# czbiohub-sf/yogo

Hardware: AMD Instinct MI355X
Metric: training images/sec (772x1032 gray) (higher is better)
Workload: dtype bf16; 1 GPU; BASELINE configs[2]: full train step (fwd+loss+bwd+clamp+AdamW), base_model, 772x1032x1 uint8, 7 classes; per_gpu_batch=128, global_batch=128, parallelism=dp1

## Files before the change

include/yogo_hip.h:

```cpp
#ifndef YOGO_HIP_H
#define YOGO_HIP_H

#include <stddef.h>

#ifdef __cplusplus
extern "C" {
#endif

typedef void* yogo_stream_t;

const char* yogo_hip_last_error(void);
int yogo_hip_abi_version(void);
int yogo_hip_launch_log(int enable);
int yogo_hip_launch_log_read(char* buf, size_t cap, size_t* needed);


int yogo_conv_packed_bytes(int Cin, int Cout, int ksize, int stride, int mode, size_t* bytes);
int yogo_conv_pack_f32(const float* w_oihw, float* packed, int Cin, int Cout, int ksize, int stride, int mode,
                       yogo_stream_t stream);
int yogo_conv2d_fwd_stats_shape(int B, int Cin, int Cout, int IH, int IW, int ksize, int stride, int* rows, int* mpad);
int yogo_conv2d_fwd_f32(const float* in, const float* packed, const float* bias, float* out, float* out_pre,
                        const float* chan_scale, float* stats_part, int B, int Cin, int Cout, int IH, int IW, int ksize,
                        int stride, int act, yogo_stream_t stream);
int yogo_conv2d_dgrad_f32(const float* dy, const float* packed_dgrad, float* dx, const float* act_ref, int ref_act,
// ... 22 lines not shown
                const float* beta, int act, float* dgamma, float* dbeta, float* part, float* sums, int B, int C, int HW,
                int training, float clip, yogo_stream_t stream);
int yogo_partials_reduce(float* part, int rows, int N, float clip, float* out, yogo_stream_t stream);
int yogo_channel_sum(const float* g, int B, int C, int HW, float clip, float* out, yogo_stream_t stream);

int yogo_decode_fwd(const float* raw, float* out, const float* cxs, const float* cys, int B, int P, int Sy, int Sx,
                    float anchor_w, float anchor_h, float width_multiplier, float height_multiplier, int inference,
                    yogo_stream_t stream);
int yogo_decode_bwd(const float* raw, const float* out, const float* gout, float* graw, int B, int P, int Sy, int Sx,
                    int inference, yogo_stream_t stream);

int yogo_decode_bwd_bf16(const float* raw, const float* out, const float* gout, void* graw8c, int B, int P, int Sy, int Sx,
                         int inference, yogo_stream_t stream);

int yogo_loss_workspace_bytes(int B, int Sy, int Sx, size_t* bytes);
int yogo_loss_fwd_bwd(const float* pred, const float* label, float* grad, float* loss_out, void* workspace, int B, int P,
                      int Sy, int Sx, float no_obj_weight, float iou_weight, float classify_weight, float label_smoothing,
                      yogo_stream_t stream);

int yogo_decode_loss_bwd_bf16(const float* raw, const float* label, const float* cxs, const float* cys, void* graw8c, float* loss_out,
                              void* workspace, int B, int P, int Sy, int Sx, float anchor_w, float anchor_h, float width_multiplier,
                              float height_multiplier, float no_obj_weight, float iou_weight, float classify_weight,
                              float label_smoothing, yogo_stream_t stream);

int yogo_format_preds_workspace_bytes(int B, int Sy, int Sx, size_t* bytes);
int yogo_format_preds_batched(const float* pred, float* out_rows, long long* out_cells, int* out_count, void* workspace,
                              int B, int P, int Sy, int Sx, int cap, double obj_thresh, double iou_thresh, int box_format,
                              double min_class_confidence_threshold, yogo_stream_t stream);
int yogo_decode_format_preds_batched(const float* raw, const float* cxs, const float* cys, float* out_rows, long long* out_cells,
                                     int* out_count, void* workspace, int B, int P, int Sy, int Sx, int cap, float anchor_w,
                                     float anchor_h, float width_multiplier, float height_multiplier, int inference,
                                     double obj_thresh, double iou_thresh, int box_format, double min_class_confidence_threshold,
                                     yogo_stream_t stream);
int yogo_head1x1_decode_fwd_bf16(const void* x, const void* packed, const float* bias, float* out, const float* cxs, const float* cys,
                                 int B, int Cin, int P, int Sy, int Sx, float anchor_w, float anchor_h, float width_multiplier,
                                 float height_multiplier, int inference, yogo_stream_t stream);

int yogo_match_workspace_bytes(int B, int Sy, int Sx, int cap, size_t* bytes);
int yogo_match_preds_labels_batched(const float* rows, const int* counts, const float* labels, int* meta, int* pair_label,
                                    int* pair_pred, int* un_label, int* un_pred, float* lab_out, void* workspace, int B, int P, int Sy,
                                    int Sx, int cap, yogo_stream_t stream);
int yogo_match_gather(const float* rows, const float* lab_out, const int* meta, const int* pair_label, const int* pair_pred,
                      const int* un_label, const int* un_pred, float* preds, float* labels, float* missed, float* extra, int B, int P,
                      int cap, long long K, long long Km, long long Ke, yogo_stream_t stream);
int yogo_metrics_state_layout(int C, int T, int nbins, long long* offsets);
int yogo_metrics_accumulate(const float* rows, const float* lab_out, const int* meta, const int* pair_label, const int* pair_pred,
// ... 182 lines not shown
```

yogo_amd/csrc/decode_loss.hip:

```cpp
#include "head_math.h"

#define MAX_CLASSES 64

__global__ __launch_bounds__(256) void decode_fwd_kernel(const float* __restrict__ raw, float* __restrict__ out,
                                                         const float* __restrict__ cxs, const float* __restrict__ cys,
                                                         float inv_sx, float inv_sy, float anchor_w, float anchor_h,
                                                         float wmul, float hmul, int P, int cells, int inference) {
  const int b = blockIdx.y;
  const int cell = blockIdx.x * 256 + threadIdx.x;
  if (cell >= cells) return;
  const float* r = raw + (size_t)b * P * cells + cell;
  float* o = out + (size_t)b * P * cells + cell;
  const float t0 = r[0], t1 = r[(size_t)cells], t2 = r[(size_t)2 * cells], t3 = r[(size_t)3 * cells], t4 = r[(size_t)4 * cells];
  o[0] = hm_centre(inv_sx, t0, cxs[cell]);
  o[(size_t)cells] = hm_centre(inv_sy, t1, cys[cell]);
  o[(size_t)2 * cells] = hm_size(anchor_w, t2, wmul);
  o[(size_t)3 * cells] = hm_size(anchor_h, t3, hmul);
  o[(size_t)4 * cells] = hm_sigmoid(t4);
  const int C = P - 5;
  if (inference) {
    float mx, sum;
    hm_softmax_terms(r, cells, P, mx, sum);
    for (int c = 0; c < C; ++c) o[(size_t)(5 + c) * cells] = hm_softmax(r[(size_t)(5 + c) * cells], mx, sum);
  } else {
// ... 27 lines not shown
  }
}

__global__ __launch_bounds__(256) void decode_bwd_bf16_kernel(const float* __restrict__ raw, const float* __restrict__ out,
                                                              const float* __restrict__ gout, hm_u32x4* __restrict__ g8, float inv_sx,
                                                              float inv_sy, int P, int Pb, int cells, int inference) {
  const int b = blockIdx.y;
  const int cell = blockIdx.x * 256 + threadIdx.x;
  if (cell >= cells) return;
  const size_t base = (size_t)b * P * cells + cell;
  const float* r = raw + base;
  const float* o = out + base;
  const float* g = gout + base;
  const float dot = inference ? hm_softmax_bwd_dot(g, o, cells, P) : 0.f;
  const float s0 = hm_sigmoid(r[0]), s1 = hm_sigmoid(r[(size_t)cells]), s4 = o[(size_t)4 * cells];
  hm_store_bf16_8c(g8, b, cell, cells, P, Pb, [&](int ch) {
    const float gv = g[(size_t)ch * cells];
    if (ch == 0) return hm_centre_bwd(gv, inv_sx, s0);
    if (ch == 1) return hm_centre_bwd(gv, inv_sy, s1);
    if (ch == 2 || ch == 3) return hm_size_bwd(gv, r[(size_t)ch * cells], o[(size_t)ch * cells]);
    if (ch == 4) return hm_obj_bwd(gv, s4);
    return inference ? hm_softmax_bwd(gv, o[(size_t)ch * cells], dot) : gv;
  });
}

struct LossWeights {
  float no_obj_weight, iou_weight, classify_weight, label_smoothing, inv_batch;
};
static LossWeights loss_weights(float no_obj_weight, float iou_weight, float classify_weight, float label_smoothing, int B) {
  return {no_obj_weight, iou_weight, classify_weight, label_smoothing, 1.0f / (float)B};
}

struct LossParams {
  const float* pred;
  const float* label;
  float* grad;
  float* part;
  int B, P, cells;
  LossWeights w;
};

__global__ __launch_bounds__(256) void yogo_loss_kernel(const LossParams p) {
  const int b = blockIdx.y;
  const int cell = blockIdx.x * 256 + threadIdx.x;
  const int cells = p.cells;
  const int C = p.P - 5;
  float l_iou = 0.f, l_obj = 0.f, l_cls = 0.f;
  if (cell < cells) {
    const float* pr = p.pred + (size_t)b * p.P * cells + cell;
    const float* lb = p.label + (size_t)b * 6 * cells + cell;
    float* gr = p.grad + (size_t)b * p.P * cells + cell;
    const float m = lb[0];
    l_obj = hm_obj_term(pr[(size_t)4 * cells], m, p.w.no_obj_weight, p.w.inv_batch, gr[(size_t)4 * cells]);
// ... 3 lines not shown
                           p.w.iou_weight * p.w.inv_batch, g0, g1, g2, g3);
    gr[0] = g0;
    gr[(size_t)cells] = g1;
    gr[(size_t)2 * cells] = g2;
    gr[(size_t)3 * cells] = g3;
    if (m != 0.f) {
      HmCeTerms ce;
      l_cls = hm_ce_cell(pr, cells, lb[(size_t)5 * cells], p.P, m, p.w.label_smoothing, p.w.classify_weight, p.w.inv_batch, ce);
      for (int c = 0; c < C; ++c) gr[(size_t)(5 + c) * cells] = hm_ce_grad(pr[(size_t)(5 + c) * cells], c, C, p.w.label_smoothing, ce);
    } else {
      for (int c = 0; c < C; ++c) gr[(size_t)(5 + c) * cells] = 0.f;
    }
  }
  hm_block_sum3(l_iou, l_obj, l_cls, p.part, b);
}

struct FusedParams {
  const float* raw;
  const float* label;
  const float *cxs, *cys;
  hm_u32x4* g8;
  float* part;
  int B, P, Pb, cells;
  float inv_sx, inv_sy, anchor_w, anchor_h, wmul, hmul;
  LossWeights w;
};

__global__ __launch_bounds__(256) void decode_loss_bwd_bf16_kernel(const FusedParams p) {
  const int b = blockIdx.y;
  const int cell = blockIdx.x * 256 + threadIdx.x;
  const int cells = p.cells;
  const int C = p.P - 5;
  float l_iou = 0.f, l_obj = 0.f, l_cls = 0.f;
  if (cell < cells) {
    const float* r = p.raw + (size_t)b * p.P * cells + cell;
    const float* lb = p.label + (size_t)b * 6 * cells + cell;
    const float t0 = r[0], t1 = r[(size_t)cells], t2 = r[(size_t)2 * cells], t3 = r[(size_t)3 * cells], t4 = r[(size_t)4 * cells];
    const float s0 = hm_sigmoid(t0), s1 = hm_sigmoid(t1);
    const float pcx = hm_centre(p.inv_sx, t0, p.cxs[cell]);
    const float pcy = hm_centre(p.inv_sy, t1, p.cys[cell]);
    const float pw = hm_size(p.anchor_w, t2, p.wmul);
    const float ph = hm_size(p.anchor_h, t3, p.hmul);
    const float po = hm_sigmoid(t4);
    const float m = lb[0];
    float gobj, g0 = 0.f, g1 = 0.f, g2 = 0.f, g3 = 0.f;
    l_obj = hm_obj_term(po, m, p.w.no_obj_weight, p.w.inv_batch, gobj);
    HmCeTerms ce{};
    if (m != 0.f) {
      l_iou = hm_ciou_cell(pcx, pcy, pw, ph, lb, cells, p.w.iou_weight * p.w.inv_batch, g0, g1, g2, g3);
      l_cls = hm_ce_cell(r, cells, lb[(size_t)5 * cells], p.P, m, p.w.label_smoothing, p.w.classify_weight, p.w.inv_batch, ce);
    }
    hm_store_bf16_8c(p.g8, b, cell, cells, p.P, p.Pb, [&](int ch) {
      if (ch == 0) return hm_centre_bwd(g0, p.inv_sx, s0);
      if (ch == 1) return hm_centre_bwd(g1, p.inv_sy, s1);
      if (ch == 2) return hm_size_bwd(g2, t2, pw);
      if (ch == 3) return hm_size_bwd(g3, t3, ph);
      if (ch == 4) return hm_obj_bwd(gobj, po);
      return m != 0.f ? hm_ce_grad(r[(size_t)ch * cells], ch - 5, C, p.w.label_smoothing, ce) : 0.f;
    });
  }
  hm_block_sum3(l_iou, l_obj, l_cls, p.part, b);
}

__global__ __launch_bounds__(256) void yogo_loss_finalize_kernel(const float* __restrict__ part, int rows, float iou_weight,
                                                                 float classify_weight, float inv_batch,
                                                                 float* __restrict__ out) {
  __shared__ double sh[3][4];
  double s[3] = {0.0, 0.0, 0.0};
  for (int r = threadIdx.x; r < rows; r += 256)
    for (int k = 0; k < 3; ++k) s[k] += (double)part[(size_t)r * 3 + k];
  const int lane = threadIdx.x & 63, wave = threadIdx.x >> 6;
  for (int k = 0; k < 3; ++k) {
    s[k] = wave_sum_d(s[k]);
    if (lane == 0) sh[k][wave] = s[k];
  }
  __syncthreads();
  if (threadIdx.x == 0) {
    const float iou = (float)(iou_weight * (sh[0][0] + sh[0][1] + sh[0][2] + sh[0][3]) * inv_batch);
    const float obj = (float)((sh[1][0] + sh[1][1] + sh[1][2] + sh[1][3]) * inv_batch);
    const float cls = (float)(classify_weight * (sh[2][0] + sh[2][1] + sh[2][2] + sh[2][3]) * inv_batch);
    out[0] = obj + iou + cls;
    out[1] = iou;
    out[2] = obj;
    out[3] = cls;
  }
}

extern "C" int yogo_decode_fwd(const float* raw, float* out, const float* cxs, const float* cys, int B, int P, int Sy,
                               int Sx, float anchor_w, float anchor_h, float width_multiplier, float height_multiplier,
                               int inference, hipStream_t stream) {
  YOGO_CHECK_ARG(raw && out && cxs && cys, "decode_fwd: null pointer");
  YOGO_CHECK_ARG(B >= 0 && P > 5 && P - 5 <= MAX_CLASSES && Sy > 0 && Sx > 0 && B <= 65535, "decode_fwd: bad shape");
  if (B == 0) return YOGO_OK;
  const int cells = Sy * Sx;
  yogo_launch_log("decode_fwd_kernel | B=%d cells=%d P=%d inference=%d", B, cells, P, inference);
  hipLaunchKernelGGL(decode_fwd_kernel, dim3(cdiv(cells, 256), B), dim3(256), 0, stream, raw, out, cxs, cys,
                     (float)(1.0 / Sx), (float)(1.0 / Sy), anchor_w, anchor_h, width_multiplier, height_multiplier, P, cells,
                     inference);
  YOGO_CHECK_LAUNCH("decode_fwd");
  return YOGO_OK;
}

extern "C" int yogo_decode_bwd(const float* raw, const float* out, const float* gout, float* graw, int B, int P, int Sy,
                               int Sx, int inference, hipStream_t stream) {
  YOGO_CHECK_ARG(raw && out && gout && graw, "decode_bwd: null pointer");
  YOGO_CHECK_ARG(B >= 0 && P > 5 && Sy > 0 && Sx > 0 && B <= 65535, "decode_bwd: bad shape");
  if (B == 0) return YOGO_OK;
  const int cells = Sy * Sx;
// ... 27 lines not shown
  YOGO_CHECK_ARG(pred && label && grad && loss_out && workspace, "loss_fwd_bwd: null pointer");
  YOGO_CHECK_ARG(B > 0 && B <= 65535 && P > 5 && P - 5 <= MAX_CLASSES && Sy > 0 && Sx > 0, "loss_fwd_bwd: bad shape");
  LossParams p{};
  p.pred = pred; p.label = label; p.grad = grad; p.part = reinterpret_cast<float*>(workspace);
  p.B = B; p.P = P; p.cells = Sy * Sx;
  p.w = loss_weights(no_obj_weight, iou_weight, classify_weight, label_smoothing, B);
  const int nb = cdiv(p.cells, 256);
  hipLaunchKernelGGL(yogo_loss_kernel, dim3(nb, B), dim3(256), 0, stream, p);
  hipLaunchKernelGGL(yogo_loss_finalize_kernel, dim3(1), dim3(256), 0, stream, p.part, B * nb, iou_weight, classify_weight,
                     p.w.inv_batch, loss_out);
  YOGO_CHECK_LAUNCH("loss_fwd_bwd");
  return YOGO_OK;
}

extern "C" int yogo_decode_loss_bwd_bf16(const float* raw, const float* label, const float* cxs, const float* cys, void* graw8c, float* loss_out,
                                         void* workspace, int B, int P, int Sy, int Sx, float anchor_w, float anchor_h, float width_multiplier,
                                         float height_multiplier, float no_obj_weight, float iou_weight, float classify_weight,
                                         float label_smoothing, hipStream_t stream) {
  YOGO_CHECK_ARG(raw && label && cxs && cys && graw8c && loss_out && workspace, "decode_loss_bwd_bf16: null pointer");
  YOGO_CHECK_ARG(B > 0 && B <= 65535 && P > 5 && P - 5 <= MAX_CLASSES && Sy > 0 && Sx > 0, "decode_loss_bwd_bf16: bad shape");
  FusedParams p{};
  p.raw = raw; p.label = label; p.cxs = cxs; p.cys = cys; p.g8 = reinterpret_cast<hm_u32x4*>(graw8c); p.part = reinterpret_cast<float*>(workspace);
  p.B = B; p.P = P; p.Pb = ((P + 15) / 16) * 2; p.cells = Sy * Sx;
  p.inv_sx = (float)(1.0 / Sx); p.inv_sy = (float)(1.0 / Sy); p.anchor_w = anchor_w; p.anchor_h = anchor_h; p.wmul = width_multiplier; p.hmul = height_multiplier;
  p.w = loss_weights(no_obj_weight, iou_weight, classify_weight, label_smoothing, B);
  const int nb = cdiv(p.cells, 256);
  hipLaunchKernelGGL(decode_loss_bwd_bf16_kernel, dim3(nb, B), dim3(256), 0, stream, p);
  hipLaunchKernelGGL(yogo_loss_finalize_kernel, dim3(1), dim3(256), 0, stream, p.part, B * nb, iou_weight, classify_weight, p.w.inv_batch, loss_out);
  YOGO_CHECK_LAUNCH("decode_loss_bwd_bf16");
  return YOGO_OK;
}
```

yogo_amd/csrc/head_math.h:

```cpp
#pragma once
#include "common.h"

typedef __bf16 hm_bf16x8 __attribute__((ext_vector_type(8)));
typedef unsigned int hm_u32x4 __attribute__((ext_vector_type(4)));

__device__ __forceinline__ float hm_sigmoid(float x) { return 1.0f / (1.0f + expf(-x)); }

__device__ __forceinline__ float hm_centre(float inv_s, float t, float c) { return inv_s * hm_sigmoid(t) + c; }
__device__ __forceinline__ float hm_size(float anchor, float t, float mul) { return anchor * expf(fminf(t, 80.f)) * mul; }
__device__ __forceinline__ void hm_softmax_terms(const float* col, size_t stride, int P, float& mx, float& sum) {
  const int C = P - 5;
  mx = -INFINITY;
  for (int c = 0; c < C; ++c) mx = fmaxf(mx, col[(size_t)(5 + c) * stride]);
  sum = 0.f;
  for (int c = 0; c < C; ++c) sum += expf(col[(size_t)(5 + c) * stride] - mx);
}
__device__ __forceinline__ float hm_softmax(float x, float mx, float sum) { return expf(x - mx) / sum; }

__device__ __forceinline__ float hm_centre_bwd(float g, float inv_s, float s) { return g * (inv_s * (s * (1.f - s))); }
__device__ __forceinline__ float hm_size_bwd(float g, float t, float o) { return t <= 80.f ? g * o : 0.f; }
__device__ __forceinline__ float hm_obj_bwd(float g, float s4) { return g * (s4 * (1.f - s4)); }
__device__ __forceinline__ float hm_softmax_bwd_dot(const float* g, const float* o, size_t stride, int P) {
  const int C = P - 5;
  float dot = 0.f;
// ... 91 lines not shown
  int tgt;
};
__device__ __forceinline__ float hm_ce_cell(const float* col, size_t stride, float cls, int P, float m, float ls, float classify_weight,
                                            float inv_batch, HmCeTerms& t) {
  const int C = P - 5;
  t.tgt = (int)cls;
  float sum;
  hm_softmax_terms(col, stride, P, t.mx, sum);
  t.lsum = logf(sum);
  float nll_t = 0.f, nll_sum = 0.f;
  for (int c = 0; c < C; ++c) {
    const float lp = log_softmax_(col[(size_t)(5 + c) * stride], t.mx, t.lsum);
    nll_sum -= lp;
    if (c == t.tgt) nll_t = -lp;
  }
  t.scl = m * classify_weight * inv_batch;
  return m * ((1.f - ls) * nll_t + (ls / (float)C) * nll_sum);
}
__device__ __forceinline__ float hm_ce_grad(float x, int c, int C, float ls, const HmCeTerms& t) {
  const float sm = expf(log_softmax_(x, t.mx, t.lsum));
  return t.scl * (sm - (c == t.tgt ? (1.f - ls) : 0.f) - ls / (float)C);
}

__device__ __forceinline__ void hm_block_sum3(float l_iou, float l_obj, float l_cls, float* part, int b) {
  __shared__ float sh[3][4];
  l_iou = wave_sum(l_iou);
  l_obj = wave_sum(l_obj);
  l_cls = wave_sum(l_cls);
  const int lane = threadIdx.x & 63, wave = threadIdx.x >> 6;
  if (lane == 0) {
    sh[0][wave] = l_iou;
    sh[1][wave] = l_obj;
    sh[2][wave] = l_cls;
  }
  __syncthreads();
  if (threadIdx.x < 3) {
    const int k = threadIdx.x;
    part[((size_t)b * gridDim.x + blockIdx.x) * 3 + k] = sh[k][0] + sh[k][1] + sh[k][2] + sh[k][3];
  }
}
```

yogo_amd/engine.py:

```python
from __future__ import annotations

import threading
import weakref
from dataclasses import dataclass, field
from typing import Dict, List, Optional, Tuple

import torch
from torch import nn

from yogo_amd import _hip

ACT_NONE, ACT_LEAKY, ACT_SILU = 0, 1, 2


@dataclass
class Layer:
    conv: nn.Conv2d
    bn: Optional[nn.BatchNorm2d] = None
    act: int = ACT_NONE
    drop: Optional[nn.Dropout2d] = None

    @property
    def cin(self) -> int:
        return self.conv.in_channels
# ... 304 lines not shown
                    act_ref = None
                dx = torch.empty(B, L.cin, IH, IW, dtype=torch.float32, device=dev)
                pk = self._packed(i, 1)
                mw_tag = 20 if L.s == 2 else (4 if L.cin > 64 else (2 if L.cin > 32 else 1))
                self._tick("dgrad", i, 2.0 * B * L.cout * L.cin * L.k * L.k * OH * OW, mw=mw_tag)
                _hip.call("yogo_conv2d_dgrad_f32", g, pk, dx, act_ref, ref_act, Sp.mask, B, L.cin, L.cout, IH, IW, L.k, L.s, st)
                self._tock()
                g = dx
        bb = self.backbone_ref()
        return [grads.get(id(p)) for p in bb.parameters()]



def _blocks(c: int) -> int:
    return ((c + 15) // 16) * 2


_FUSE_LAYER0_BWD = True
_L0_NO_Z = True
_WGRAD_DEFER_REDUCE = True
_L01_FUSE_BWD = True
_PAIR_FWD = True
_HEAD_BN_FUSE = True


def _packed_bf16(eng: Engine, i: int, mode: int) -> torch.Tensor:
    L = eng.layers[i]
    w = L.conv.weight
    key = (i, 10 + mode)
    buf = _pack_hit(eng, key, w)
    if buf is not None:
        return buf
    nbytes = _hip.query_size("yogo_conv_bf16_packed_bytes", L.cin, L.cout, L.k, mode)
    buf = torch.empty(nbytes, dtype=torch.uint8, device=w.device)
    _hip.call("yogo_conv_bf16_pack", _f32(w.detach()), None, buf, L.cin, L.cout, L.k, mode, _hip.stream_ptr())
    eng._pack[key] = (w._version, w.data_ptr(), buf)
    return buf


def _pack_all_bf16(eng: Engine) -> None:
    jobs = [(i, mode) for i in range(1, len(eng.layers)) for mode in (0, 2 if (eng.layers[i].s == 2 and eng.layers[i].k == 3) else 1)]
    ws = [eng.layers[i].conv.weight for i, _ in jobs]
    if any(w.dtype != torch.float32 or not w.is_contiguous() for w in ws) or not jobs:
        return
    if all(_pack_hit(eng, (i, 10 + m), w) is not None for (i, m), w in zip(jobs, ws)):
        return
# ... 148 lines not shown

def _pair_fwd_bf16(eng: Engine, i: int, Sa: Saved, Sb: Saved, B: int, H: int, W: int, st) -> torch.Tensor:
    La, Lb = eng.layers[i], eng.layers[i + 1]
    dev = Sa.x_in.device
    OH, OW = Lb.out_hw(H, W)
    bias_a = _f32(La.conv.bias.detach()) if La.conv.bias is not None else None
    bias_b = _f32(Lb.conv.bias.detach()) if Lb.conv.bias is not None else None
    pk_a, pk_b = _packed_bf16(eng, i, 0), _packed_bf16(eng, i + 1, 0)
    y1 = torch.empty(B, _blocks(La.cout), H, W, 8, dtype=torch.bfloat16, device=dev)
    y2 = torch.empty(B, _blocks(Lb.cout), OH, OW, 8, dtype=torch.bfloat16, device=dev)
    Sa.signs = torch.empty(_hip.query_size("yogo_bf16_signs_bytes", B, La.cout, H, W), dtype=torch.uint8, device=dev)
    Sb.signs = torch.empty(_hip.query_size("yogo_bf16_signs_bytes", B, Lb.cout, OH, OW), dtype=torch.uint8, device=dev)
    flops = 2.0 * B * 9 * (La.cout * La.cin * H * W + Lb.cout * Lb.cin * OH * OW)
    nbytes = B * 16 * ((_blocks(La.cin) + _blocks(La.cout)) * H * W + _blocks(Lb.cout) * OH * OW)
    eng._tick("fwd", i, flops, mw=30, nbytes=nbytes)
    _hip.call("yogo_conv2d_fwd_bf16_signs_pair", Sa.x_in, pk_a, bias_a, y1, Sa.signs, Sa.mask, pk_b, bias_b, y2, Sb.signs, Sb.mask,
              B, La.cin, La.cout, Lb.cout, H, W, ACT_LEAKY, st)
    eng._tock()
    Sb.x_in = y1
    Sa.y, Sb.y = y1, y2
    return y2


def forward_bf16_train(eng: Engine, x: torch.Tensor) -> Tuple[torch.Tensor, List[Saved]]:
    _check_bf16_train_input(eng, x)
    dev, st, B = x.device, _hip.stream_ptr(), x.shape[0]
    _pack_all_bf16(eng)
    masks = _dropout_masks(eng, B, dev)
    cur = x.contiguous() if x.dtype == torch.uint8 else _f32(x)
    H, W = int(cur.shape[2]), int(cur.shape[3])
    saved: List[Saved] = []
    n = len(eng.layers)
    paired = -1
    for i, L in enumerate(eng.layers):
        if i == paired:
            H, W = L.out_hw(H, W)
            continue
        OH, OW = L.out_hw(H, W)
        if OH <= 0 or OW <= 0:
            raise RuntimeError(f"yogo_amd: image too small at layer {i}")
        last = i == n - 1
        has_bn = L.bn is not None
        if L.act == ACT_SILU and not has_bn and (i == 0 or last):
            raise RuntimeError("yogo_amd: bf16 training of a first / last SiLU block without BatchNorm is not implemented (use fp32)")
        bias = _f32(L.conv.bias.detach()) if L.conv.bias is not None else None
        S = Saved(x_in=cur, mask=masks.get(i))
        bn_train = has_bn and (L.bn.training or L.bn.running_mean is None)
        if _PAIR_FWD and _pair_fwd_eligible(eng, i, B, H, W):
            OH2, OW2 = eng.layers[i + 1].out_hw(OH, OW)
            if OH2 <= 0 or OW2 <= 0:
                raise RuntimeError(f"yogo_amd: image too small at layer {i + 1}")
            S2 = Saved(x_in=None, mask=masks.get(i + 1))
            cur = _pair_fwd_bf16(eng, i, S, S2, B, H, W, st)
            saved += [S, S2]
            paired = i + 1
            H, W = OH, OW
            continue
        if (i == 0 and has_bn and S.mask is None and not last and cur.dtype == torch.uint8
                and _hip.lib().yogo_conv_first_mfma_supported(0, L.cin, L.cout, H, W, L.s)):
            cur = _first_mfma_fwd_bf16(eng, L, S, bias, bn_train, B, H, W, st)
        else:
            cur = _layer_fwd_bf16(eng, i, L, S, bias, bn_train, last, B, H, W, st)
        saved.append(S)
        H, W = OH, OW
    return cur, saved


def backward_bf16_train(eng: Engine, saved: List[Saved], graw: torch.Tensor,
                        grad_out: Optional[Dict[int, torch.Tensor]] = None, on_layer=None,
                        trace: Optional[dict] = None, flush_layers=None, stop_at: int = 0) -> List[Optional[torch.Tensor]]:
    n = len(eng.layers)
    if not 0 <= stop_at < n:
        raise ValueError(f"yogo_amd: stop_at {stop_at} is not a layer of this {n}-layer network")
    st, dev, clip = _hip.stream_ptr(), graw.device, float(eng.clip)
    grads: Dict[int, torch.Tensor] = {}

    def dst(param: torch.Tensor) -> torch.Tensor:
        if grad_out is not None and id(param) in grad_out:
            return grad_out[id(param)]
        return torch.empty(param.shape, dtype=torch.float32, device=dev)

    queued_ws: List[torch.Tensor] = []
    wq = _wgrad_queue() if (_WGRAD_DEFER_REDUCE and (on_layer is None or flush_layers is not None)) else None
    flush_at = frozenset(flush_layers) if flush_layers is not None else frozenset()
    if wq is not None:
        _hip.call("yogo_wgrad_reduce_queue_reset", wq)
    if graw.dtype == torch.bfloat16 and graw.ndim == 5:
        g = graw
        B = g.shape[0]
    else:
        graw = _f32(graw)
        B, P, Sy, Sx = graw.shape
        g = torch.empty(B, _blocks(P), Sy, Sx, 8, dtype=torch.bfloat16, device=dev)
# ... 100 lines not shown
            if trace is not None:
                trace[("dz", i)] = g.clone()
        dw = dst(L.conv.weight)
        db = dst(L.conv.bias) if L.conv.bias is not None else None
        if fuse0:
            wgrad_first_bn(L, S, g, fused01, dw, IH, IW)
        elif fuse01:
            fused01 = wgrad_dgrad_first(L, S, g, dw, db, IH, IW, OH, OW)
        elif i == 0:
            _first_wgrad("yogo_conv_first_wgrad_bf16g", L, S.x_in, g, dw, db, clip, st)
        else:
            wgrad(i, L, S, g, dw, db, IH, IW, OH, OW)
        if db is not None:
            grads[id(L.conv.bias)] = db
        grads[id(L.conv.weight)] = dw
        if on_layer is not None:
            if wq is not None and i in flush_at:
                _hip.call("yogo_wgrad_reduce_flush", wq, st)
            on_layer(i)
        if fuse01:
            g = None
        elif head_below:
            head_g = (g, _f32(L.conv.weight.detach()).reshape(L.cout, L.cin), L.cout)
        elif i > stop_at:
            g = dgrad(i, L, g, Sp, act_ref, ref_act, IH, IW, OH, OW)
    if wq is not None:
        _hip.call("yogo_wgrad_reduce_flush", wq, st)
    bb = eng.backbone_ref()
    return [grads.get(id(p)) for p in bb.parameters()]


_WGRAD_QUEUE = None


def _wgrad_queue() -> int:
    global _WGRAD_QUEUE
    if _WGRAD_QUEUE is None:
        import ctypes
        h = ctypes.c_void_p(0)
        _hip.call("yogo_wgrad_reduce_queue_create", ctypes.addressof(h))
        _WGRAD_QUEUE = int(h.value)
    return _WGRAD_QUEUE


_ENGINES: "weakref.WeakKeyDictionary[nn.Module, Engine]" = weakref.WeakKeyDictionary()

# ... 246 lines not shown
```

yogo_amd/train.py:

```python
from __future__ import annotations

import ctypes
import math
from typing import Dict, List, Optional, Tuple

import torch
import torch.distributed as dist

from yogo_amd import _hip
from yogo_amd.engine import get_engine
from yogo_amd.model import YOGO
from yogo_amd.yogo_loss import YOGOLoss

_FUSED_DECODE_LOSS = True


def cosine_lr(step: int, base_lr: float, t_max: int, eta_min: float) -> float:
    return eta_min + (base_lr - eta_min) * (1 + math.cos(math.pi * step / t_max)) / 2


class FlatParams:

    def __init__(self, module: torch.nn.Module):
        self.params: List[torch.nn.Parameter] = [p for p in module.parameters()]
# ... 224 lines not shown
            b.copy_(flat[off:off + n].view(b.shape).to(b.dtype))
            off += n
        off = 0
        for b in cnt:
            n = b.numel()
            b.copy_(icnt[off:off + n].view(b.shape).to(b.dtype))
            off += n
        self.engine.generation += 1

    @torch.no_grad()
    def step(self, imgs: torch.Tensor, labels: torch.Tensor) -> torch.Tensor:
        m = self.model
        _hip.require_cuda(imgs, "imgs")
        _hip.require_cuda(labels, "labels")
        with torch.cuda.device(imgs.device):
            st = _hip.stream_ptr()
            eng = self.engine
            eng.clip = m._clip
            self.flat.check_homed()
            if imgs.ndim == 3:
                imgs = imgs[None]
            if not imgs.is_floating_point() and imgs.dtype != torch.uint8:
                imgs = imgs.float()
            if self.half:
                from yogo_amd.engine import backward_bf16_train, forward_bf16_train

                raw, saved = forward_bf16_train(eng, imgs)
                if self.trace is not None:
                    self.trace["saved"], self.trace["raw"] = saved, raw
            else:
                raw, saved = eng.forward(imgs, need_grad=True)
            B, P, Sy, Sx = raw.shape
            aw, ah, wm, hm = m._decode_scalars()
            cxs, cys = _hip.grid_buffers(m._Cxs, m._Cys, Sy, Sx, raw.device)
            L = self.loss
            out = torch.empty(4, dtype=torch.float32, device=raw.device)
            ws = torch.empty(_hip.query_size("yogo_loss_workspace_bytes", B, Sy, Sx) // 4, dtype=torch.float32, device=raw.device)
            lab = labels if (labels.dtype == torch.float32 and labels.is_contiguous()) else labels.contiguous().float()
            hook = self._on_layer_done if self.world > 1 else None
            flush = (self.split_layer,) if hook is not None else None
            lw = (float(L.no_obj_weight), float(L.iou_weight), float(L.classify_weight), float(L.label_smoothing))

            def decode_and_loss():
                pred, gpred = torch.empty_like(raw), torch.empty_like(raw)
                _hip.call("yogo_decode_fwd", raw, pred, cxs, cys, B, P, Sy, Sx, aw, ah, wm, hm, int(bool(m.inference)), st)
                _hip.call("yogo_loss_fwd_bwd", pred, lab, gpred, out, ws, B, P, Sy, Sx, *lw, st)
                return pred, gpred

            g8 = torch.empty(B, ((P + 15) // 16) * 2, Sy, Sx, 8, dtype=torch.bfloat16, device=raw.device) if self.half else None
            if self.half and not m.inference and _FUSED_DECODE_LOSS:
                _hip.call("yogo_decode_loss_bwd_bf16", raw, lab, cxs, cys, g8, out, ws, B, P, Sy, Sx, aw, ah, wm, hm, *lw, st)
                backward_bf16_train(eng, saved, g8, grad_out=self.flat.grad_views, on_layer=hook, trace=self.trace, flush_layers=flush)
            elif self.half:
                pred, gpred = decode_and_loss()
                _hip.call("yogo_decode_bwd_bf16", raw, pred, gpred, g8, B, P, Sy, Sx, int(bool(m.inference)), st)
                backward_bf16_train(eng, saved, g8, grad_out=self.flat.grad_views, on_layer=hook, trace=self.trace, flush_layers=flush)
            else:
                pred, gpred = decode_and_loss()
                graw = torch.empty_like(raw)
                _hip.call("yogo_decode_bwd", raw, pred, gpred, graw, B, P, Sy, Sx, int(bool(m.inference)), st)
                eng.backward(saved, graw, grad_out=self.flat.grad_views, on_layer=hook)
            started = self.split_off if (self.overlap and self._pending) else self.flat.total
            self.exchange_begin(0, started)
            scale = self.exchange_end()
            lr = self.current_lr()
            self.global_step += 1
            _hip.call("yogo_adamw_step", self.flat.flat, self.flat.grad, self.flat.exp_avg, self.flat.exp_avg_sq, self.flat.total,
                      self.global_step, lr, self.betas[0], self.betas[1], self.eps, self.wd, scale, st)
            eng.invalidate_packed()
            self.last_loss = out
            return out

    def loss_components(self) -> Dict[str, float]:
# ... 3 lines not shown
```

Before: 10970 images/s.

## Fuse head 1x1 conv forward, decode+loss backward, and head dgrad into one kernel

Adds a single head-sweep kernel that computes the final 1x1 conv with MFMA, keeps raw predictions in shared memory, runs decode+loss+grad per cell, then immediately computes the head's input gradient with the leaky-ReLU mask from the bf16 input. The training step skips the separate head forward, the fp32 raw round trip and the separate dgrad launch when the head is eligible. This removes the global-memory write and reread of raw predictions and several launches, at the cost of a more complex kernel with high register use and a new eligibility path.

```diff
diff --git a/include/yogo_hip.h b/include/yogo_hip.h
--- a/include/yogo_hip.h
+++ b/include/yogo_hip.h
@@ -68,6 +68,11 @@
                               void* workspace, int B, int P, int Sy, int Sx, float anchor_w, float anchor_h, float width_multiplier,
                               float height_multiplier, float no_obj_weight, float iou_weight, float classify_weight,
                               float label_smoothing, yogo_stream_t stream);
+int yogo_head_sweep_bf16_eligible(int B, int Cin, int P, int Sy, int Sx);
+int yogo_head_sweep_bf16(const void* y, const void* packed_fwd, const void* packed_dgrad, const float* bias, const float* label,
+                         const float* cxs, const float* cys, void* graw8c, void* dx, float* raw, float* loss_out, void* workspace, int B,
+                         int Cin, int P, int Sy, int Sx, float anchor_w, float anchor_h, float width_multiplier, float height_multiplier,
+                         float no_obj_weight, float iou_weight, float classify_weight, float label_smoothing, yogo_stream_t stream);
 
 int yogo_format_preds_workspace_bytes(int B, int Sy, int Sx, size_t* bytes);
 int yogo_format_preds_batched(const float* pred, float* out_rows, long long* out_cells, int* out_count, void* workspace,
diff --git a/yogo_amd/csrc/decode_loss.hip b/yogo_amd/csrc/decode_loss.hip
--- a/yogo_amd/csrc/decode_loss.hip
+++ b/yogo_amd/csrc/decode_loss.hip
@@ -73,13 +73,6 @@
     if (ch == 4) return hm_obj_bwd(gv, s4);
     return inference ? hm_softmax_bwd(gv, o[(size_t)ch * cells], dot) : gv;
   });
-}
-
-struct LossWeights {
-  float no_obj_weight, iou_weight, classify_weight, label_smoothing, inv_batch;
-};
-static LossWeights loss_weights(float no_obj_weight, float iou_weight, float classify_weight, float label_smoothing, int B) {
-  return {no_obj_weight, iou_weight, classify_weight, label_smoothing, 1.0f / (float)B};
 }
 
 struct LossParams {
@@ -129,7 +122,7 @@
   hm_u32x4* g8;
   float* part;
   int B, P, Pb, cells;
-  float inv_sx, inv_sy, anchor_w, anchor_h, wmul, hmul;
+  HmDecodeConsts d;
   LossWeights w;
 };
 
@@ -137,34 +130,12 @@
   const int b = blockIdx.y;
   const int cell = blockIdx.x * 256 + threadIdx.x;
   const int cells = p.cells;
-  const int C = p.P - 5;
   float l_iou = 0.f, l_obj = 0.f, l_cls = 0.f;
   if (cell < cells) {
     const float* r = p.raw + (size_t)b * p.P * cells + cell;
     const float* lb = p.label + (size_t)b * 6 * cells + cell;
-    const float t0 = r[0], t1 = r[(size_t)cells], t2 = r[(size_t)2 * cells], t3 = r[(size_t)3 * cells], t4 = r[(size_t)4 * cells];
-    const float s0 = hm_sigmoid(t0), s1 = hm_sigmoid(t1);
-    const float pcx = hm_centre(p.inv_sx, t0, p.cxs[cell]);
-    const float pcy = hm_centre(p.inv_sy, t1, p.cys[cell]);
-    const float pw = hm_size(p.anchor_w, t2, p.wmul);
-    const float ph = hm_size(p.anchor_h, t3, p.hmul);
-    const float po = hm_sigmoid(t4);
-    const float m = lb[0];
-    float gobj, g0 = 0.f, g1 = 0.f, g2 = 0.f, g3 = 0.f;
-    l_obj = hm_obj_term(po, m, p.w.no_obj_weight, p.w.inv_batch, gobj);
-    HmCeTerms ce{};
-    if (m != 0.f) {
-      l_iou = hm_ciou_cell(pcx, pcy, pw, ph, lb, cells, p.w.iou_weight * p.w.inv_batch, g0, g1, g2, g3);
-      l_cls = hm_ce_cell(r, cells, lb[(size_t)5 * cells], p.P, m, p.w.label_smoothing, p.w.classify_weight, p.w.inv_batch, ce);
-    }
-    hm_store_bf16_8c(p.g8, b, cell, cells, p.P, p.Pb, [&](int ch) {
-      if (ch == 0) return hm_centre_bwd(g0, p.inv_sx, s0);
-      if (ch == 1) return hm_centre_bwd(g1, p.inv_sy, s1);
-      if (ch == 2) return hm_size_bwd(g2, t2, pw);
-      if (ch == 3) return hm_size_bwd(g3, t3, ph);
-      if (ch == 4) return hm_obj_bwd(gobj, po);
-      return m != 0.f ? hm_ce_grad(r[(size_t)ch * cells], ch - 5, C, p.w.label_smoothing, ce) : 0.f;
-    });
+    hm_decode_loss_bwd_cell(r, cells, lb, cells, p.cxs[cell], p.cys[cell], p.P, p.d, p.w, l_iou, l_obj, l_cls,
+                            [&](auto v) { hm_store_bf16_8c(p.g8, b, cell, cells, p.P, p.Pb, v); });
   }
   hm_block_sum3(l_iou, l_obj, l_cls, p.part, b);
 }
@@ -191,6 +162,12 @@
     out[2] = obj;
     out[3] = cls;
   }
+}
+
+int launch_loss_finalize(const float* part, int rows, float iou_weight, float classify_weight, float inv_batch, float* loss_out, hipStream_t stream) {
+  hipLaunchKernelGGL(yogo_loss_finalize_kernel, dim3(1), dim3(256), 0, stream, part, rows, iou_weight, classify_weight, inv_batch, loss_out);
+  YOGO_CHECK_LAUNCH("loss_finalize");
+  return YOGO_OK;
 }
 
 extern "C" int yogo_decode_fwd(const float* raw, float* out, const float* cxs, const float* cys, int B, int P, int Sy,
@@ -264,7 +241,7 @@
   FusedParams p{};
   p.raw = raw; p.label = label; p.cxs = cxs; p.cys = cys; p.g8 = reinterpret_cast<hm_u32x4*>(graw8c); p.part = reinterpret_cast<float*>(workspace);
   p.B = B; p.P = P; p.Pb = ((P + 15) / 16) * 2; p.cells = Sy * Sx;
-  p.inv_sx = (float)(1.0 / Sx); p.inv_sy = (float)(1.0 / Sy); p.anchor_w = anchor_w; p.anchor_h = anchor_h; p.wmul = width_multiplier; p.hmul = height_multiplier;
+  p.d = {(float)(1.0 / Sx), (float)(1.0 / Sy), anchor_w, anchor_h, width_multiplier, height_multiplier};
   p.w = loss_weights(no_obj_weight, iou_weight, classify_weight, label_smoothing, B);
   const int nb = cdiv(p.cells, 256);
   hipLaunchKernelGGL(decode_loss_bwd_bf16_kernel, dim3(nb, B), dim3(256), 0, stream, p);
diff --git a/yogo_amd/csrc/head_math.h b/yogo_amd/csrc/head_math.h
--- a/yogo_amd/csrc/head_math.h
+++ b/yogo_amd/csrc/head_math.h
@@ -137,6 +137,46 @@
   return t.scl * (sm - (c == t.tgt ? (1.f - ls) : 0.f) - ls / (float)C);
 }
 
+struct LossWeights {
+  float no_obj_weight, iou_weight, classify_weight, label_smoothing, inv_batch;
+};
+static inline LossWeights loss_weights(float no_obj_weight, float iou_weight, float classify_weight, float label_smoothing, int B) {
+  return {no_obj_weight, iou_weight, classify_weight, label_smoothing, 1.0f / (float)B};
+}
+struct HmDecodeConsts {
+  float inv_sx, inv_sy, anchor_w, anchor_h, wmul, hmul;
+};
+template <class Emit>
+__device__ __forceinline__ void hm_decode_loss_bwd_cell(const float* r, size_t rstride, const float* lb, size_t lstride, float cx, float cy, int P,
+                                                        const HmDecodeConsts& d, const LossWeights& w, float& l_iou, float& l_obj, float& l_cls,
+                                                        Emit emit) {
+  const int C = P - 5;
+  const float t0 = r[0], t1 = r[rstride], t2 = r[2 * rstride], t3 = r[3 * rstride], t4 = r[4 * rstride];
+  const float s0 = hm_sigmoid(t0), s1 = hm_sigmoid(t1);
+  const float pcx = hm_centre(d.inv_sx, t0, cx);
+  const float pcy = hm_centre(d.inv_sy, t1, cy);
+  const float pw = hm_size(d.anchor_w, t2, d.wmul);
+  const float ph = hm_size(d.anchor_h, t3, d.hmul);
+  const float po = hm_sigmoid(t4);
+  const float m = lb[0];
+  float gobj, g0 = 0.f, g1 = 0.f, g2 = 0.f, g3 = 0.f;
+  l_obj = hm_obj_term(po, m, w.no_obj_weight, w.inv_batch, gobj);
+  HmCeTerms ce{};
+  if (m != 0.f) {
+    l_iou = hm_ciou_cell(pcx, pcy, pw, ph, lb, lstride, w.iou_weight * w.inv_batch, g0, g1, g2, g3);
+    l_cls = hm_ce_cell(r, rstride, lb[5 * lstride], P, m, w.label_smoothing, w.classify_weight, w.inv_batch, ce);
+  }
+  emit([&](int ch) {
+    if (ch == 0) return hm_centre_bwd(g0, d.inv_sx, s0);
+    if (ch == 1) return hm_centre_bwd(g1, d.inv_sy, s1);
+    if (ch == 2) return hm_size_bwd(g2, t2, pw);
+    if (ch == 3) return hm_size_bwd(g3, t3, ph);
+    if (ch == 4) return hm_obj_bwd(gobj, po);
+    return m != 0.f ? hm_ce_grad(r[(size_t)ch * rstride], ch - 5, C, w.label_smoothing, ce) : 0.f;
+  });
+}
+int launch_loss_finalize(const float* part, int rows, float iou_weight, float classify_weight, float inv_batch, float* loss_out, hipStream_t stream);
+
 __device__ __forceinline__ void hm_block_sum3(float l_iou, float l_obj, float l_cls, float* part, int b) {
   __shared__ float sh[3][4];
   l_iou = wave_sum(l_iou);
diff --git a/yogo_amd/csrc/head_sweep.hip b/yogo_amd/csrc/head_sweep.hip
--- /dev/null
+++ b/yogo_amd/csrc/head_sweep.hip
@@ -0,0 +1,165 @@
+#include "head_math.h"
+#include "bf16_dev.h"
+#include "conv_bf16_plan.h"
+
+struct HeadSweepParams {
+  const u32x4* in;
+  const u32x4* wp_fwd;
+  const u32x4* wp_dg;
+  const float* bias;
+  const float* label;
+  const float *cxs, *cys;
+  hm_u32x4* g8;
+  u32x4* dx;
+  float* raw;
+  float* part;
+  int P, plane, Mpad;
+  HmDecodeConsts d;
+  LossWeights w;
+};
+
+template <int NK>
+__global__ __launch_bounds__(256) void decode_loss_bwd_bf16_kernel_head(const HeadSweepParams p) {
+  constexpr int KB = 2 * NK;
+  constexpr int NMB = (NK + 1) / 2;
+  __shared__ float s_raw[16][256];
+  __shared__ hm_u32x4 s_g[2][256];
+  const int tid = threadIdx.x, lane = tid & 63, l31 = lane & 31, half = lane >> 5;
+  const int wave = __builtin_amdgcn_readfirstlane(tid >> 6);
+  const int b = blockIdx.y;
+  const int plane = p.plane, plane16 = plane * 16;
+  const auto rs_in = __builtin_amdgcn_make_buffer_rsrc((void*)(p.in + (size_t)b * KB * plane), (short)0, KB * plane16, RSRC_WORD3);
+  int v0[2];
+  bool ov[2];
+  u32x4 Bq[2][NK];
+#pragma unroll
+  for (int t = 0; t < 2; ++t) {
+    const int px = blockIdx.x * 256 + wave * 64 + 32 * t + l31;
+    ov[t] = px < plane;
+    v0[t] = ov[t] ? (half * plane + px) * 16 : (int)OOB;
+#pragma unroll
+    for (int kc = 0; kc < NK; ++kc) Bq[t][kc] = __builtin_bit_cast(u32x4, __builtin_amdgcn_raw_buffer_load_b128(rs_in, v0[t], (2 * kc) * plane16, 0));
+  }
+  u32x4 Aq[NK];
+#pragma unroll
+  for (int kc = 0; kc < NK; ++kc) Aq[kc] = p.wp_fwd[(2 * kc + half) * 32 + l31];
+  float bs[8];
+#pragma unroll
+  for (int i = 0; i < 8; ++i) {
+    const int ch = 8 * (i >> 2) + 4 * half + (i & 3);
+    bs[i] = (p.bias != nullptr && ch < p.P) ? p.bias[ch] : 0.f;
+  }
+  unsigned sg[2][2] = {{0u, 0u}, {0u, 0u}};
+#pragma unroll
+  for (int t = 0; t < 2; ++t) {
+    f32x16 acc;
+#pragma unroll
+    for (int r = 0; r < 16; ++r) acc[r] = 0.f;
+#pragma unroll
+    for (int kc = 0; kc < NK; ++kc)
+      acc = __builtin_amdgcn_mfma_f32_32x32x16_bf16(__builtin_bit_cast(bf16x8, Aq[kc]), __builtin_bit_cast(bf16x8, Bq[t][kc]), acc, 0, 0, 0);
+#pragma unroll
+    for (int kc = 0; kc < NK; ++kc) {
+      const bf16x8 y = __builtin_bit_cast(bf16x8, Bq[t][kc]);
+      unsigned m = 0;
+#pragma unroll
+      for (int j = 0; j < 8; ++j) m |= ((float)y[j] > 0.f ? 1u : 0u) << j;
+      sg[t][kc >> 2] |= m << (8 * (kc & 3));
+    }
+    const int cl = wave * 64 + 32 * t + l31;
+    float* ob = p.raw != nullptr ? p.raw + (size_t)b * p.P * plane + blockIdx.x * 256 + cl : nullptr;
+#pragma unroll
+    for (int i = 0; i < 8; ++i) {
+      const int ch = 8 * (i >> 2) + 4 * half + (i & 3);
+      const float v = acc[i] + bs[i];
+      s_raw[ch][cl] = v;
+      if (ob != nullptr && ov[t] && ch < p.P) ob[(size_t)ch * plane] = v;
+    }
+  }
+  __syncthreads();
+  const int cell = blockIdx.x * 256 + tid;
+  float l_iou = 0.f, l_obj = 0.f, l_cls = 0.f;
+  if (cell < plane) {
+    const float* lb = p.label + (size_t)b * 6 * plane + cell;
+    hm_decode_loss_bwd_cell(&s_raw[0][tid], 256, lb, plane, p.cxs[cell], p.cys[cell], p.P, p.d, p.w, l_iou, l_obj, l_cls,
+                            [&](auto v) { hm_store_bf16_8c(&s_g[0][0], 0, tid, 256, p.P, 2, v); });
+    p.g8[((size_t)b * 2 + 0) * plane + cell] = s_g[0][tid];
+    p.g8[((size_t)b * 2 + 1) * plane + cell] = s_g[1][tid];
+  } else {
+    s_g[0][tid] = hm_u32x4{0u, 0u, 0u, 0u};
+    s_g[1][tid] = hm_u32x4{0u, 0u, 0u, 0u};
+  }
+  hm_block_sum3(l_iou, l_obj, l_cls, p.part, b);
+  __syncthreads();
+  unsigned sm[2][2];
+#pragma unroll
+  for (int t = 0; t < 2; ++t)
+#pragma unroll
+    for (int q = 0; q < 2; ++q) {
+      const unsigned own = sg[t][q], oth = (unsigned)__shfl_xor((int)own, 32, 64);
+      sm[t][q] = half == 0 ? (own & 0x0F0F0F0Fu) | ((oth << 4) & 0xF0F0F0F0u) : ((oth >> 4) & 0x0F0F0F0Fu) | (own & 0xF0F0F0F0u);
+    }
+  u32x4 Aw[NMB];
+#pragma unroll
+  for (int mb = 0; mb < NMB; ++mb) Aw[mb] = p.wp_dg[half * p.Mpad + mb * 32 + l31];
+  const auto rs_o = __builtin_amdgcn_make_buffer_rsrc((void*)(p.dx + (size_t)b * KB * plane), (short)0, KB * plane16, RSRC_WORD3);
+#pragma unroll
+  for (int t = 0; t < 2; ++t) {
+    const u32x4 Bg = __builtin_bit_cast(u32x4, s_g[half][wave * 64 + 32 * t + l31]);
+#pragma unroll
+    for (int mb = 0; mb < NMB; ++mb) {
+      f32x16 acc;
+#pragma unroll
+      for (int r = 0; r < 16; ++r) acc[r] = 0.f;
+      acc = __builtin_amdgcn_mfma_f32_32x32x16_bf16(__builtin_bit_cast(bf16x8, Aw[mb]), __builtin_bit_cast(bf16x8, Bg), acc, 0, 0, 0);
+#pragma unroll
+      for (int gp = 0; gp < 2; ++gp) {
+        const int kc = 2 * mb + gp;
+        if (kc >= NK) continue;
+        const unsigned m = sm[t][kc >> 2] >> (8 * (kc & 3));
+        float v[8];
+#pragma unroll
+        for (int i = 0; i < 8; ++i) v[i] = acc[8 * gp + i] * ((m >> i) & 1u ? 1.f : LEAKY_SLOPE);
+        const u32x4 o = pack_unit_swap(v);
+        __builtin_amdgcn_raw_buffer_store_b128(o, rs_o, ov[t] ? v0[t] + (2 * kc) * plane16 : (int)OOB, 0, 0);
+      }
+    }
+  }
+}
+
+bool head_sweep_eligible(int B, int Cin, int P, int plane) {
+  return P >= 6 && P <= 16 && B > 0 && B <= 65535 && conv_bf16_head_fwd_eligible(Cin, P, plane, B) && (long long)B * cdiv(plane, 256) * 3 < (1ll << 31);
+}
+
+extern "C" int yogo_head_sweep_bf16_eligible(int B, int Cin, int P, int Sy, int Sx) {
+  return (Sy > 0 && Sx > 0 && (long long)Sy * Sx < (1ll << 31) && head_sweep_eligible(B, Cin, P, Sy * Sx)) ? 1 : 0;
+}
+
+extern "C" int yogo_head_sweep_bf16(const void* y, const void* packed_fwd, const void* packed_dgrad, const float* bias, const float* label,
+                                    const float* cxs, const float* cys, void* graw8c, void* dx, float* raw, float* loss_out, void* workspace, int B,
+                                    int Cin, int P, int Sy, int Sx, float anchor_w, float anchor_h, float width_multiplier, float height_multiplier,
+                                    float no_obj_weight, float iou_weight, float classify_weight, float label_smoothing, hipStream_t stream) {
+  YOGO_CHECK_ARG(y && packed_fwd && packed_dgrad && label && cxs && cys && graw8c && dx && loss_out && workspace, "head_sweep_bf16: null pointer");
+  YOGO_CHECK_ARG(yogo_head_sweep_bf16_eligible(B, Cin, P, Sy, Sx),
+                 "head_sweep_bf16: unsupported shape (6 <= P <= 16, Cin a multiple of 16 and <= 128; ask yogo_head_sweep_bf16_eligible)");
+  HeadSweepParams p{};
+  p.in = reinterpret_cast<const u32x4*>(y); p.wp_fwd = reinterpret_cast<const u32x4*>(packed_fwd); p.wp_dg = reinterpret_cast<const u32x4*>(packed_dgrad);
+  p.bias = bias; p.label = label; p.cxs = cxs; p.cys = cys; p.g8 = reinterpret_cast<hm_u32x4*>(graw8c); p.dx = reinterpret_cast<u32x4*>(dx); p.raw = raw;
+  p.part = reinterpret_cast<float*>(workspace);
+  p.P = P; p.plane = Sy * Sx; p.Mpad = bf_mpad_of(Cin);
+  p.d = {(float)(1.0 / Sx), (float)(1.0 / Sy), anchor_w, anchor_h, width_multiplier, height_multiplier};
+  p.w = loss_weights(no_obj_weight, iou_weight, classify_weight, label_smoothing, B);
+  const int nb = cdiv(p.plane, 256);
+  switch (Cin / 16) {
+#define HS_CASE(NK) \
+  case NK: hipLaunchKernelGGL((decode_loss_bwd_bf16_kernel_head<NK>), dim3(nb, B), dim3(256), 0, stream, p); break;
+    HS_CASE(1) HS_CASE(2) HS_CASE(3) HS_CASE(4) HS_CASE(5) HS_CASE(6) HS_CASE(7) HS_CASE(8)
+#undef HS_CASE
+    default: yogo_set_error("head_sweep_bf16: Cin = %d", Cin); return YOGO_ERR_ARG;
+  }
+  if (yogo_launch_log_enabled())
+    yogo_launch_log("decode_loss_bwd_bf16_kernel_head<%d> | Cin=%d P=%d plane=%d grid=%dx%d bias=%d raw=%d", Cin / 16, Cin, P, p.plane, nb, B, bias != nullptr,
+                    raw != nullptr);
+  YOGO_CHECK_LAUNCH("head_sweep_bf16");
+  return launch_loss_finalize(p.part, B * nb, iou_weight, classify_weight, p.w.inv_batch, loss_out, stream);
+}
diff --git a/yogo_amd/engine.py b/yogo_amd/engine.py
--- a/yogo_amd/engine.py
+++ b/yogo_amd/engine.py
@@ -350,6 +350,7 @@
 _L01_FUSE_BWD = True
 _PAIR_FWD = True
 _HEAD_BN_FUSE = True
+_HEAD_SWEEP = True
 
 
 def _packed_bf16(eng: Engine, i: int, mode: int) -> torch.Tensor:
@@ -544,7 +545,36 @@
     return y2
 
 
-def forward_bf16_train(eng: Engine, x: torch.Tensor) -> Tuple[torch.Tensor, List[Saved]]:
+def _head_sweep_eligible(eng: Engine, below_mask, B: int, H: int, W: int) -> bool:
+    n = len(eng.layers)
+    if n < 3:
+        return False
+    L, Lp = eng.layers[n - 1], eng.layers[n - 2]
+    if L.k != 1 or L.s != 1 or L.bn is not None or L.act != ACT_NONE or Lp.bn is not None or Lp.act != ACT_LEAKY or below_mask is not None:
+        return False
+    return bool(_hip.lib().yogo_head_sweep_bf16_eligible(B, L.cin, L.cout, H, W))
+
+
+def head_sweep_bf16(eng: Engine, saved: List[Saved], lab: torch.Tensor, cxs: torch.Tensor, cys: torch.Tensor, loss_out: torch.Tensor,
+                    ws: torch.Tensor, decode_scalars, loss_weights, want_raw: bool) -> Tuple[torch.Tensor, torch.Tensor]:
+    n = len(eng.layers)
+    L, S = eng.layers[n - 1], saved[n - 1]
+    y, dev, st = S.x_in, S.x_in.device, _hip.stream_ptr()
+    B, Sy, Sx = int(y.shape[0]), int(y.shape[2]), int(y.shape[3])
+    bias = _f32(L.conv.bias.detach()) if L.conv.bias is not None else None
+    gh = torch.empty(B, _blocks(L.cout), Sy, Sx, 8, dtype=torch.bfloat16, device=dev)
+    g = torch.empty_like(y)
+    raw = torch.empty(B, L.cout, Sy, Sx, dtype=torch.float32, device=dev) if want_raw else None
+    eng._tick("fwd", n - 1, 2.0 * 2.0 * B * L.cout * L.cin * Sy * Sx, mw=30,
+              nbytes=B * Sy * Sx * (2 * 16 * _blocks(L.cin) + 16 * _blocks(L.cout) + 6 * 4))
+    _hip.call("yogo_head_sweep_bf16", y, _packed_bf16(eng, n - 1, 0), _packed_bf16(eng, n - 1, 1), bias, lab, cxs, cys, gh, g, raw, loss_out, ws,
+              B, L.cin, L.cout, Sy, Sx, *decode_scalars, *loss_weights, st)
+    eng._tock()
+    S.y = raw
+    return gh, g
+
+
+def forward_bf16_train(eng: Engine, x: torch.Tensor, head_sweep: bool = False) -> Tuple[torch.Tensor, List[Saved]]:
     _check_bf16_train_input(eng, x)
     dev, st, B = x.device, _hip.stream_ptr(), x.shape[0]
     _pack_all_bf16(eng)
@@ -568,6 +598,9 @@
         bias = _f32(L.conv.bias.detach()) if L.conv.bias is not None else None
         S = Saved(x_in=cur, mask=masks.get(i))
         bn_train = has_bn and (L.bn.training or L.bn.running_mean is None)
+        if last and head_sweep and S.mask is None and _head_sweep_eligible(eng, masks.get(i - 1), B, H, W):
+            saved.append(S)
+            return cur, saved
         if _PAIR_FWD and _pair_fwd_eligible(eng, i, B, H, W):
             OH2, OW2 = eng.layers[i + 1].out_hw(OH, OW)
             if OH2 <= 0 or OW2 <= 0:
@@ -590,7 +623,8 @@
 
 def backward_bf16_train(eng: Engine, saved: List[Saved], graw: torch.Tensor,
                         grad_out: Optional[Dict[int, torch.Tensor]] = None, on_layer=None,
-                        trace: Optional[dict] = None, flush_layers=None, stop_at: int = 0) -> List[Optional[torch.Tensor]]:
+                        trace: Optional[dict] = None, flush_layers=None, stop_at: int = 0,
+                        head_dx: Optional[torch.Tensor] = None) -> List[Optional[torch.Tensor]]:
     n = len(eng.layers)
     if not 0 <= stop_at < n:
         raise ValueError(f"yogo_amd: stop_at {stop_at} is not a layer of this {n}-layer network")
@@ -737,6 +771,8 @@
             g = None
         elif head_below:
             head_g = (g, _f32(L.conv.weight.detach()).reshape(L.cout, L.cin), L.cout)
+        elif i == n - 1 and head_dx is not None:
+            g = head_dx
         elif i > stop_at:
             g = dgrad(i, L, g, Sp, act_ref, ref_act, IH, IW, OH, OW)
     if wq is not None:
diff --git a/yogo_amd/train.py b/yogo_amd/train.py
--- a/yogo_amd/train.py
+++ b/yogo_amd/train.py
@@ -270,15 +270,22 @@
                 imgs = imgs[None]
             if not imgs.is_floating_point() and imgs.dtype != torch.uint8:
                 imgs = imgs.float()
+            swept = False
             if self.half:
-                from yogo_amd.engine import backward_bf16_train, forward_bf16_train
-
-                raw, saved = forward_bf16_train(eng, imgs)
-                if self.trace is not None:
+                from yogo_amd import engine as E
+                from yogo_amd.engine import backward_bf16_train, forward_bf16_train, head_sweep_bf16
+
+                want_sweep = bool(not m.inference and _FUSED_DECODE_LOSS and E._HEAD_SWEEP)
+                raw, saved = forward_bf16_train(eng, imgs, head_sweep=want_sweep)
+                swept = want_sweep and saved[-1].y is None
+                if self.trace is not None and not swept:
                     self.trace["saved"], self.trace["raw"] = saved, raw
             else:
                 raw, saved = eng.forward(imgs, need_grad=True)
-            B, P, Sy, Sx = raw.shape
+            if swept:
+                B, P, Sy, Sx = int(raw.shape[0]), eng.layers[-1].cout, int(raw.shape[2]), int(raw.shape[3])
+            else:
+                B, P, Sy, Sx = raw.shape
             aw, ah, wm, hm = m._decode_scalars()
             cxs, cys = _hip.grid_buffers(m._Cxs, m._Cys, Sy, Sx, raw.device)
             L = self.loss
@@ -295,8 +302,13 @@
                 _hip.call("yogo_loss_fwd_bwd", pred, lab, gpred, out, ws, B, P, Sy, Sx, *lw, st)
                 return pred, gpred
 
-            g8 = torch.empty(B, ((P + 15) // 16) * 2, Sy, Sx, 8, dtype=torch.bfloat16, device=raw.device) if self.half else None
-            if self.half and not m.inference and _FUSED_DECODE_LOSS:
+            g8 = torch.empty(B, ((P + 15) // 16) * 2, Sy, Sx, 8, dtype=torch.bfloat16, device=raw.device) if (self.half and not swept) else None
+            if swept:
+                g8, gin = head_sweep_bf16(eng, saved, lab, cxs, cys, out, ws, (aw, ah, wm, hm), lw, want_raw=self.trace is not None)
+                if self.trace is not None:
+                    self.trace["saved"], self.trace["raw"] = saved, saved[-1].y
+                backward_bf16_train(eng, saved, g8, grad_out=self.flat.grad_views, on_layer=hook, trace=self.trace, flush_layers=flush, head_dx=gin)
+            elif self.half and not m.inference and _FUSED_DECODE_LOSS:
                 _hip.call("yogo_decode_loss_bwd_bf16", raw, lab, cxs, cys, g8, out, ws, B, P, Sy, Sx, aw, ah, wm, hm, *lw, st)
                 backward_bf16_train(eng, saved, g8, grad_out=self.flat.grad_views, on_layer=hook, trace=self.trace, flush_layers=flush)
             elif self.half:
```

Result: no change. 11030 images/s, median of 6 (+0.5%).
